# andi611/ZeroSpeech-TTS-without-T

Hardware: AMD Instinct MI355X
Metric: mel-frames/sec (train_ae, seg_len=128, enc_size=1024) (higher is better)
Workload: dtype bf16; 1 GPU; train_ae english hps seg_len=128 enc_size=1024 emb_size=1024 n_speakers=102 F=513, batch=256/GPU, dropout+Gumbel on, fwd+bwd+clip+Adam; global_batch=256, parallelism=dp1

## Files before the change

### include/zs_amd.h

```cpp
#ifndef ZS_AMD_H
#define ZS_AMD_H
#include <stddef.h>
#include <stdint.h>

#ifdef __cplusplus
extern "C" {
#endif

#define ZS_ABI_VERSION 1

enum { ZS_F32 = 0, ZS_BF16 = 1 };
enum { ZS_OK = 0, ZS_EINVAL = -1, ZS_ELAUNCH = -2, ZS_EWORKSPACE = -3 };
enum { ZS_PAD_ZERO = 0, ZS_PAD_REFLECT = 1 };
enum { ZS_ACT_NONE = 0, ZS_ACT_LRELU = 1, ZS_ACT_SIGMOID = 2, ZS_ACT_TANH = 3 };
enum { ZS_STORE_ROWS = 0, ZS_STORE_SPLIT2 = 1 };
enum { ZS_RES_NONE = 0, ZS_RES_IDENTITY = 1, ZS_RES_AVGPOOL2 = 2, ZS_RES_UPSAMPLE2 = 3 };

int zs_abi_version(void);
const char* zs_last_error(void);
int zs_set_option(const char* key, int value);
int zs_get_option(const char* key);

typedef struct {
  int32_t dtype;
// ... 175 lines not shown
  void* out; int64_t ldo; int32_t out_col;
  void* gates;
  float* work; size_t work_bytes;
  int32_t whh_interleaved;
  uint32_t* status;
  const float* bcast_vec; int64_t bcast_ld; const int64_t* bcast_idx; int32_t bcast_col;
  int32_t dir1_forward;
} ZsGruFwd;
size_t zs_gru_work_bytes(int32_t B, int32_t H);
int zs_gru_fwd(const ZsGruFwd* p, void* stream);
int zs_gru_check(const float* work, int32_t B, int32_t H, void* stream);

typedef struct {
  int32_t dtype;
  void* x; int64_t ld; int32_t col0, cols;
  int32_t B, T; const int32_t* lengths;
} ZsRowsReverse;
int zs_rows_reverse(const ZsRowsReverse* p, void* stream);
typedef struct {
  int32_t dtype;
  int32_t B, T, H;
  const void* dout; int64_t ldd; int32_t dout_col;
  const void* out; int64_t ldo; int32_t out_col;
  const void* gates;
  const void* whh_t; int64_t ldw; int32_t n_pad; int64_t w_gstride;
  void* dgi; int64_t ldgi;
  void* dgh; int64_t ldgh;
  float* work; size_t work_bytes;
  uint32_t* status;
} ZsGruBwd;
int zs_gru_bwd(const ZsGruBwd* p, void* stream);
enum { ZS_GRU_PATH_WIDE = 0, ZS_GRU_PATH_PERSIST = 1, ZS_GRU_PATH_STEP_FUSED = 2, ZS_GRU_PATH_STEP_GEMM = 3 };
int zs_gru_path(int32_t pass, int32_t dtype, int32_t B, int32_t T, int32_t H, int32_t whh_interleaved, int32_t wide_aligned);

typedef struct {
  int32_t dtype;
  const float* x_dec; int64_t ld_dec;
  const float* x; int64_t ldx;
  int64_t rows; int32_t F;
  void* dlogits; int64_t ldg; int32_t fill_cols;
  float* partial; float* loss_out; float grad_scale;
} ZsL1Loss;
int zs_l1_loss(const ZsL1Loss* p, void* stream);

int zs_sqnorm(const float* g, int64_t n, double* partial, float* out_sq, void* stream);

typedef struct {
  float* p; float* g; float* m; float* v; int64_t n;
  float lr, beta1, beta2, eps, bc1, bc2;
  const float* sumsq; float max_norm; int32_t write_clipped_grad;
  const int32_t* step_ptr;
  float grad_scale;
  int32_t max_blocks;
  float* ema;
  float ema_decay;
} ZsAdam;
int zs_adam_clip(const ZsAdam* p, void* stream);

int zs_sqnorm_stage1(const float* g, int64_t n, double* partial, void* stream);

enum { ZS_APJ_WEIGHT = 0, ZS_APJ_VECTOR = 1, ZS_APJ_RANGE = 2 };
typedef struct {
  void* dst; int64_t ldw; int64_t dst_elems;
  int32_t transpose, inner_pad, row_offset, col_offset, parity;
  int32_t vlen, src_offset, src_stride;
  const int32_t* row_inv;
// ... 284 lines not shown
```

### zerospeech-tts-without-t_amd/_lib.py

```python
import ctypes
import os
import re

_PKG = os.path.dirname(os.path.abspath(__file__))
_ROOT = os.path.dirname(_PKG)
HEADER = os.path.join(_ROOT, 'include', 'zs_amd.h')
_SAN = os.environ.get('ZS_SANITIZE', '').strip()
LIB_PATH = os.environ.get('ZS_LIB_PATH') or os.path.join(_PKG, 'libzs_amd.%s.so' % _SAN if _SAN else 'libzs_amd.so')

_CTYPES = {
    'int32_t': ctypes.c_int32, 'int64_t': ctypes.c_int64, 'uint32_t': ctypes.c_uint32, 'uint64_t': ctypes.c_uint64,
    'float': ctypes.c_float, 'double': ctypes.c_double, 'size_t': ctypes.c_size_t, 'int': ctypes.c_int,
}


def _strip_comments(text):
    return re.sub(r'/\*.*?\*/', ' ', text, flags=re.S)


def _make_struct(name, fields):
    return type(name, (ctypes.Structure,), {'_fields_': fields})


def parse_header(path=HEADER):
# ... 38 lines not shown


_STRUCT_FIELDS, FUNCTIONS, ENUMS = parse_header()
globals().update(ENUMS)

STRUCTS = {name: _make_struct(name, fields) for name, fields in _STRUCT_FIELDS.items()}
for _fields in _STRUCT_FIELDS.values():
    for _, _ct in _fields:
        _el = getattr(_ct, '_type_', None)
        if isinstance(_el, type) and issubclass(_el, ctypes.Structure):
            STRUCTS[_el.__name__] = _el

_lib = None


class ZsError(RuntimeError):
    pass


def lib():
    global _lib
    if _lib is None:
        if not os.path.exists(LIB_PATH):
            raise ZsError('libzs_amd.so is missing at %s: run `python -c "import __graft_entry__ as g; g.build()"` '
                          '(the HIP extension is mandatory; there is no fallback path)' % LIB_PATH)
        L = ctypes.CDLL(LIB_PATH)
        L.zs_last_error.restype = ctypes.c_char_p
        L.zs_abi_version.restype = ctypes.c_int
        L.zs_gemm_wgrad_workspace_bytes.restype = ctypes.c_size_t
        L.zs_gemm_wgrad_path.argtypes = [ctypes.c_void_p, ctypes.c_void_p, ctypes.c_void_p]
        L.zs_gru_work_bytes.restype = ctypes.c_size_t
        L.zs_gru_work_bytes.argtypes = [ctypes.c_int32, ctypes.c_int32]
        L.zs_gru_check.argtypes = [ctypes.c_void_p, ctypes.c_int32, ctypes.c_int32, ctypes.c_void_p]
        L.zs_sqnorm.argtypes = [ctypes.c_void_p, ctypes.c_int64, ctypes.c_void_p, ctypes.c_void_p, ctypes.c_void_p]
        L.zs_sqnorm_stage1.argtypes = [ctypes.c_void_p, ctypes.c_int64, ctypes.c_void_p, ctypes.c_void_p]
        L.zs_adam_pack_tiles.argtypes = [ctypes.c_void_p]
        L.zs_adam_pack.argtypes = [ctypes.c_void_p, ctypes.c_void_p, ctypes.c_void_p, ctypes.c_int32, ctypes.c_void_p, ctypes.c_int32,
                                   ctypes.c_void_p]
        L.zs_get_option.argtypes = [ctypes.c_char_p]
        L.zs_step_counters.argtypes = [ctypes.c_void_p, ctypes.c_void_p, ctypes.c_void_p]
        L.zs_set_option.argtypes = [ctypes.c_char_p, ctypes.c_int]
        L.zs_pre_mel.argtypes = [ctypes.c_void_p, ctypes.c_void_p, ctypes.c_void_p, ctypes.c_int64, ctypes.c_int32, ctypes.c_float,
                                 ctypes.c_float, ctypes.c_void_p]
        V, I32, I64, F32 = ctypes.c_void_p, ctypes.c_int32, ctypes.c_int64, ctypes.c_float
        L.zs_row_moments_workspace.restype = ctypes.c_size_t
        L.zs_row_moments_workspace.argtypes = [I32, I32, I32]
        L.zs_in2d_finalize.argtypes = [V, V, V, V, I64, I32, F32, V]
        L.zs_in2d_stats.argtypes = [I32, V, I64, I32, I32, I32, F32, V, V, V, ctypes.c_size_t, V]
        L.zs_lerp_rows.argtypes = [V, V, V, V, I32, I64, V]
        L.zs_gp_penalty.argtypes = [V, I32, I64, F32, V, V, V, V]
        L.zs_gen_combine_fwd.argtypes = [V, V, I64, V, I64, I32, I32, V]
        L.zs_l1_plain.argtypes = [V, V, I64, F32, V, V, V, V]
        L.zs_host_fetch.argtypes = [V, V, ctypes.c_size_t, I32, V]
        L.zs_griffin_lim.argtypes = [ctypes.c_void_p, ctypes.c_void_p, ctypes.c_void_p, ctypes.c_int32, ctypes.c_void_p]
        L.zs_conv1_wgrad_workspace.restype = ctypes.c_size_t
        L.zs_conv1_wgrad_workspace.argtypes = []
        L.zs_gl_chains_used.argtypes = []
        L.zs_gl_chains_used.restype = ctypes.c_int
        if hasattr(L, 'zs_gl_denormalize'):
            L.zs_gl_denormalize.argtypes = [ctypes.c_void_p, ctypes.c_void_p, ctypes.c_int64, ctypes.c_void_p]
        if hasattr(L, 'zs_gl_deemphasis'):
            L.zs_gl_deemphasis.argtypes = [ctypes.c_void_p, ctypes.c_int64, ctypes.c_void_p, ctypes.c_int32, ctypes.c_float,
                                           ctypes.c_void_p]
        L.zs_gl_frame_mse.argtypes = [ctypes.c_void_p, ctypes.c_int64, ctypes.c_void_p, ctypes.c_int32, ctypes.c_int32, ctypes.c_int32,
                                      ctypes.c_void_p, ctypes.c_int64, ctypes.c_void_p]
        L.zs_trim_workspace_bytes.restype = ctypes.c_size_t
# ... 111 lines not shown
```

### zerospeech-tts-without-t_amd/csrc/zs_gru.hip

```cpp
#include <stdlib.h>
#include <string.h>

#include <atomic>

#include "zs_common.h"

extern "C" size_t zs_gru_work_bytes(int32_t B, int32_t H);

namespace {

constexpr size_t GRU_WORK_HDR = 256;

constexpr int NTG = 256;

struct GateFwdArgs {
  const void* gi; int64_t ldgi;
  const float* gh;
  const float* bhh; int64_t bhh_gstride;
  float* hstate;
  void* out; int64_t ldo; int out_col;
  void* gates;
  int B, T, H, step;
  int dir1_forward;
};
// ... 657 lines not shown
      }
      if constexpr (NCH > 0) {
        const unsigned poff = (unsigned)(s & 1) * par_bytes;
#pragma unroll
        for (int i = 0; i < NCH; ++i) g4[i] = load16_sc1(hx_rs, poff + ch_off[i]);
      }
      unsigned char* const nimg = &himg[(s + 1) & 1][0];
#pragma unroll
      for (int i = 0; i < 4; ++i) *reinterpret_cast<bf16_t*>(nimg + (4 * q + i) * PITCH + unit * 2) = f2bf(hv[i]);
    }
#pragma unroll
    for (int i = 0; i < 4; ++i) {
      out_s[s & 1][0][4 * q + i][ul] = f2bf(hv[i]);
      out_s[s & 1][1][4 * q + i][ul] = f2bf(rg[i]); out_s[s & 1][2][4 * q + i][ul] = f2bf(zg[i]);
      out_s[s & 1][3][4 * q + i][ul] = f2bf(ng[i]); out_s[s & 1][4][4 * q + i][ul] = f2bf(hn[i]);
    }
  }
  __syncthreads();
  copy_out((T_ - 1) & 1, fwd_t ? T_ - 1 : 0);
}

struct GruPersistBwdArgs {
  const void* dout; int64_t ldd; int dout_col;
  const void* out; int64_t ldo; int out_col;
  const void* gates;
  const void* whh_t; int64_t ldw; int64_t w_gstride;
  void* dgi; int64_t ldgi;
  void* dgh; int64_t ldgh;
  unsigned long long* dx;
  unsigned* err;
  unsigned* status;
  unsigned spin_limit;
  int B, T, H, rows_pad;
};

constexpr int BNT = 4;
template <typename T, int PERB>
__global__ __launch_bounds__(256) void gru_persist_bwd_kernel(const GruPersistBwdArgs a) {
  constexpr int KSTEP = Frag16<T>::KSTEP;
  constexpr int EPL = 16 / (int)sizeof(T);
  constexpr int GPE = 4 / (int)sizeof(T);
  __shared__ float part[4][BNT][4][64];
  const int tid = threadIdx.x, lane = tid & 63, wave = tid >> 6;
  const int q = lane >> 4, r = lane & 15;
  const int d = blockIdx.z, H = a.H, T_ = a.T;
  const int m0 = blockIdx.y * 16;
  const int gpr = 3 * H / GPE;
  const int64_t par_stride = (int64_t)a.rows_pad * gpr;
  unsigned long long* dx_d = a.dx + (int64_t)d * 2 * par_stride;

  uint4 fb[PERB][BNT];
  {
    const T* Wrow = (const T*)a.whh_t + (int64_t)d * a.w_gstride + (int64_t)(blockIdx.x * 16 * BNT + r) * a.ldw + q * EPL;
#pragma unroll
    for (int u = 0; u < PERB; ++u)
#pragma unroll
      for (int c = 0; c < BNT; ++c) fb[u][c] = *reinterpret_cast<const uint4*>(Wrow + (int64_t)(16 * c) * a.ldw + (wave * PERB + u) * KSTEP);
  }
  const bool rvalid = (m0 + r) < a.B;
  const unsigned long long* Ag = dx_d + (int64_t)(m0 + r) * gpr + (q * EPL + wave * PERB * KSTEP) / GPE;
  const int eu2 = tid & 31, e_row = tid >> 5;
  const int j = blockIdx.x * 16 * BNT + 2 * eu2;
  const int hh = (2 * eu2) >> 4, cc = (2 * eu2) & 15;
  float dhd[2][2] = {{0.f, 0.f}, {0.f, 0.f}};
  bool dead = false;

// ... 93 lines not shown
          Pair<T>::publish(xr, j, (unsigned)(s + 1), dr_pre[pz][0], dr_pre[pz][1]);
          Pair<T>::publish(xr, H + j, (unsigned)(s + 1), dz_pre[pz][0], dz_pre[pz][1]);
          Pair<T>::publish(xr, 2 * H + j, (unsigned)(s + 1), dnr[pz][0], dnr[pz][1]);
        }
      }
    }
#pragma unroll
    for (int pz = 0; pz < 2; ++pz) {
      const int b = m0 + e_row + 8 * pz;
      if (b < a.B) {
        const int64_t row = (int64_t)b * T_ + t;
        T* gi = (T*)a.dgi + row * a.ldgi + (int64_t)d * 3 * H + j;
        T* gh = (T*)a.dgh + row * a.ldgh + (int64_t)d * 3 * H + j;
        Pair<T>::st(gi, dr_pre[pz][0], dr_pre[pz][1]); Pair<T>::st(gi + H, dz_pre[pz][0], dz_pre[pz][1]); Pair<T>::st(gi + 2 * H, dn_pre[pz][0], dn_pre[pz][1]);
        Pair<T>::st(gh, dr_pre[pz][0], dr_pre[pz][1]); Pair<T>::st(gh + H, dz_pre[pz][0], dz_pre[pz][1]); Pair<T>::st(gh + 2 * H, dnr[pz][0], dnr[pz][1]);
      }
    }
    __syncthreads();
  }
}

template <int KS>
__global__ __launch_bounds__(256) void gru_wide_bwd_kernel(const GruPersistBwdArgs a) {
  constexpr int H = 32 * KS;
  constexpr int NCH = 3 * (KS / 2 - 1);
  constexpr int NCHA = NCH > 0 ? NCH : 1;
  constexpr int CPR = (H - 64) / 4;
  constexpr int PITCH = 3 * H * 2 + 16;
  __shared__ __attribute__((aligned(16))) unsigned char gimg[2][16 * PITCH];
  __shared__ __attribute__((aligned(16))) bf16_t in_s[2][6][16][64];
  __shared__ __attribute__((aligned(16))) bf16_t out_s[2][4][16][64];
  const int tid = threadIdx.x, lane = tid & 63, wave = tid >> 6;
  const int q = lane >> 4, r = lane & 15;
  const int d = blockIdx.z, T_ = a.T;
  const int m0 = blockIdx.y * 16;
  const int u_wg = blockIdx.x * 64;
  const int ul = wave * 16 + r;
  const int unit = u_wg + ul;
  constexpr int gpr = 3 * H / 2;
  const int64_t par_stride = (int64_t)a.rows_pad * gpr;
  unsigned long long* dx_d = a.dx + (int64_t)d * 2 * par_stride;
  const gru_rsrc_t dx_rs = make_buffer_rsrc(dx_d, (unsigned)(2 * par_stride * 8));
  const unsigned par_bytes = (unsigned)(par_stride * 8);

  uint4 fb[3 * KS];
  {
    const bf16_t* Wb = (const bf16_t*)a.whh_t + (int64_t)d * a.w_gstride + (int64_t)(u_wg + wave * 16 + r) * a.ldw + q * 8;
#pragma unroll
    for (int kk = 0; kk < 3 * KS; ++kk) fb[kk] = *reinterpret_cast<const uint4*>(Wb + kk * 32);
  }
  int ch_row[NCHA], ch_col[NCHA];
  unsigned ch_off[NCHA];
  bool ch_valid[NCHA];
#pragma unroll
  for (int i = 0; i < NCH; ++i) {
    const int c = tid + 256 * i;
    const int row = c / (3 * CPR), rem = c - row * (3 * CPR), g = rem / CPR, cu = (rem - g * CPR) * 4;
    ch_row[i] = row; ch_col[i] = g * H + (cu < u_wg ? cu : cu + 64);
    ch_valid[i] = (m0 + row) < a.B;
    ch_off[i] = (unsigned)(((int64_t)(m0 + row) * gpr + (ch_col[i] >> 1)) * 8);
  }
  auto in_src = [&](int id, int s_) -> const bf16_t* {
    const int arr = id >> 7, rem = id & 127, row = rem >> 3, c = rem & 7;
    const int b = min(m0 + row, a.B - 1);
    const int t = d == 0 ? T_ - 1 - s_ : s_;
    if (arr < 4) return (const bf16_t*)a.gates + (((int64_t)b * T_ + t) * 2 + d) * 4 * H + arr * H + u_wg + 8 * c;
    if (arr == 4) return (const bf16_t*)a.dout + ((int64_t)b * T_ + t) * a.ldd + a.dout_col + d * H + u_wg + 8 * c;
    const int tp = s_ < T_ - 1 ? (d == 0 ? t - 1 : t + 1) : t;
    return (const bf16_t*)a.out + ((int64_t)b * T_ + tp) * a.ldo + a.out_col + d * H + u_wg + 8 * c;
// ... 104 lines not shown
      dnr[i] = dn_pre[i] * r_;
    }
    ZS_PT(3)
    if (s + 1 < T_) {
      unsigned long long* dx_w = dx_d + (int64_t)(s & 1) * par_stride;
#pragma unroll
      for (int i = 0; i < 4; ++i) {
        const float n0 = __shfl_xor(dr_pre[i], 1, 64), n1 = __shfl_xor(dz_pre[i], 1, 64), n2 = __shfl_xor(dnr[i], 1, 64);
        const int b = m0 + 4 * q + i;
        if (!(lane & 1) && b < a.B) {
          unsigned long long* xr = dx_w + (int64_t)b * gpr;
          store_granule(xr + (unit >> 1), (unsigned)(s + 1), Pair<bf16_t>::pack(dr_pre[i], n0));
          store_granule(xr + ((H + unit) >> 1), (unsigned)(s + 1), Pair<bf16_t>::pack(dz_pre[i], n1));
          store_granule(xr + ((2 * H + unit) >> 1), (unsigned)(s + 1), Pair<bf16_t>::pack(dnr[i], n2));
        }
      }
      unsigned char* const nimg = &gimg[(s + 1) & 1][0];
#pragma unroll
      for (int i = 0; i < 4; ++i) {
        bf16_t* row = reinterpret_cast<bf16_t*>(nimg + (4 * q + i) * PITCH);
        row[unit] = f2bf(dr_pre[i]); row[H + unit] = f2bf(dz_pre[i]); row[2 * H + unit] = f2bf(dnr[i]);
      }
    }
#pragma unroll
    for (int i = 0; i < 4; ++i) {
      out_s[s & 1][0][4 * q + i][ul] = f2bf(dr_pre[i]); out_s[s & 1][1][4 * q + i][ul] = f2bf(dz_pre[i]);
      out_s[s & 1][2][4 * q + i][ul] = f2bf(dn_pre[i]); out_s[s & 1][3][4 * q + i][ul] = f2bf(dnr[i]);
    }
    ZS_PT(4)
  }
  __syncthreads();
  copy_out((T_ - 1) & 1, T_ - 1);
#ifdef ZS_GRU_PROFILE
  if (blockIdx.x == 2 && blockIdx.y == 3 && d == 0 && tid == 0) {
    long long* o = reinterpret_cast<long long*>(a.err) + 8;
    for (int k = 0; k < 5; ++k) o[k] = pc[k];
  }
#endif
#undef ZS_PT
}

inline unsigned gate_blocks(int64_t total) {
  int64_t b = (total + NTG - 1) / NTG;
  if (b > 2048) b = 2048;
  return (unsigned)(b < 1 ? 1 : b);
}

size_t gru_hx_bytes(int B, int H, int es) {
  const size_t rows = (size_t)((B + 16 * RB - 1) / (16 * RB)) * 16 * RB;
  return (size_t)2 * 2 * rows * ((size_t)H * es / 4) * 8;
}

Knob g_gru_persist("gru_persist", "ZS_GRU_PERSIST", 1, knob_flag);
Knob g_gru_wide("gru_wide", "ZS_GRU_WIDE", 1, knob_flag);
Knob g_gru_spin_limit("gru_spin_limit", "ZS_GRU_SPIN_LIMIT", (int)GRU_SPIN_LIMIT);
int64_t gru_resident_limit() {
  static std::atomic<int> cus{0};
  int c = cus.load(std::memory_order_relaxed);
  if (c == 0) {
    int dev = 0; hipDeviceProp_t prop;
    if (hipGetDevice(&dev) == hipSuccess && hipGetDeviceProperties(&prop, dev) == hipSuccess) c = prop.multiProcessorCount;
    if (c <= 0) c = 256;
    cus.store(c, std::memory_order_relaxed);
  }
  return c;
}

bool gru_wide_aligned(const ZsGruFwd* p) {
  return (p->out_col % 8) == 0 && (p->ldo % 8) == 0 && (p->ldgi % 8) == 0 && ((uintptr_t)p->out % 16) == 0 && ((uintptr_t)p->gi % 16) == 0 &&
         (!p->gates || ((uintptr_t)p->gates % 16) == 0) && (!p->bcast_vec || (p->bcast_col % 8) == 0);
}
bool gru_wide_aligned(const ZsGruBwd* p) {
  return (p->dout_col % 8) == 0 && (p->out_col % 8) == 0 && (p->ldd % 8) == 0 && (p->ldo % 8) == 0 && (p->ldgi % 8) == 0 && (p->ldgh % 8) == 0 &&
         (((uintptr_t)p->dout | (uintptr_t)p->out | (uintptr_t)p->gates | (uintptr_t)p->dgi | (uintptr_t)p->dgh) % 16) == 0;
}

struct GruPlan {
  int path;
  int per;
  int rb;
  unsigned spin_limit;
};

GruPlan gru_plan(int pass, int dtype, int B, int T, int H, bool whh_interleaved, bool wide_aligned) {
  const bool bwd = pass != 0;
  if (H % 32 != 0 || (!bwd && !whh_interleaved)) return {ZS_GRU_PATH_STEP_GEMM, 0, 0, 0};
  const bool persist = g_gru_persist.get() != 0 && T > 1, wide = g_gru_wide.get() != 0;
  const unsigned spin = (unsigned)g_gru_spin_limit.get();
  const int nrb16 = (B + 15) / 16, nrb = (B + 16 * RB - 1) / (16 * RB);
  const int kstep = dtype == ZS_F32 ? 16 : 32;
  if (persist && wide && dtype == ZS_BF16 && (H == 128 || H == 256 || H == 512) && (int64_t)(H / 64) * nrb16 * 2 <= gru_resident_limit() &&
      wide_aligned)
    return {ZS_GRU_PATH_WIDE, 0, nrb16, spin};
  if (!bwd) {
    const int per = (H % (4 * kstep) == 0) ? H / (4 * kstep) : 0;
    if (persist && (per == 1 || per == 2 || per == 4) && (int64_t)(H / 32) * nrb * 2 <= gru_resident_limit())
      return {ZS_GRU_PATH_PERSIST, per, nrb, spin};
    return {ZS_GRU_PATH_STEP_FUSED, 0, nrb, spin};
  }
  const int perb = ((3 * H) % (4 * kstep) == 0 && H % (16 * BNT) == 0) ? (3 * H) / (4 * kstep) : 0;
  if (persist && (perb == 3 || perb == 6 || perb == 12) && (int64_t)(H / (16 * BNT)) * nrb16 * 2 <= gru_resident_limit())
    return {ZS_GRU_PATH_PERSIST, perb, nrb16, spin};
  return {ZS_GRU_PATH_STEP_FUSED, 0, nrb, spin};
}

GruPlan gru_fwd_plan(const ZsGruFwd* p) {
  return gru_plan(0, p->dtype, p->B, p->T, p->H, p->whh_interleaved != 0, gru_wide_aligned(p));
}

GruPlan gru_bwd_plan(const ZsGruBwd* p) {
  return gru_plan(1, p->dtype, p->B, p->T, p->H, true, gru_wide_aligned(p));
}

}

extern "C" size_t zs_gru_work_bytes(int32_t B, int32_t H) {
  const size_t steps = (size_t)2 * (size_t)B * (size_t)(5 * H) * sizeof(float) + 256;
  const size_t hx = gru_hx_bytes(B, 3 * H, 4) + 256;
  return steps > hx ? steps : hx;
}

extern "C" int zs_gru_check(const float* work, int32_t B, int32_t H, void* stream) {
  ZS_REQUIRE(work && B > 0 && H > 0, "zs_gru_check: bad args");
  unsigned v = 0;
  if (hipMemcpyAsync(&v, reinterpret_cast<const char*>(work), sizeof(v), hipMemcpyDeviceToHost,
                     (hipStream_t)stream) != hipSuccess || hipStreamSynchronize((hipStream_t)stream) != hipSuccess) {
    zs_set_error("zs_gru_check: copy failed");
    return ZS_ELAUNCH;
  }
  if (v != 0) { zs_set_error("zs_gru_check: a persistent GRU workgroup timed out waiting for its group (results are invalid)"); return ZS_ELAUNCH; }
  return ZS_OK;
}

extern "C" int zs_gru_path(int32_t pass, int32_t dtype, int32_t B, int32_t T, int32_t H, int32_t whh_interleaved, int32_t wide_aligned) {
  ZS_REQUIRE(pass == 0 || pass == 1, "zs_gru_path: pass 0 (zs_gru_fwd) or 1 (zs_gru_bwd)");
  ZS_REQUIRE(dtype == ZS_F32 || dtype == ZS_BF16, "zs_gru_path: bad dtype");
  ZS_REQUIRE(B > 0 && T > 0 && H > 0 && H % 8 == 0, "zs_gru_path: sizes");
  const GruPlan pl = gru_plan(pass, dtype, B, T, H, whh_interleaved != 0, wide_aligned != 0);
  return pl.path | (pl.per << 8);
}

extern "C" int zs_gru_fwd(const ZsGruFwd* p, void* stream) {
  ZS_REQUIRE(p && p->gi && p->whh && p->bhh && p->out && p->work, "zs_gru_fwd: null operand");
  ZS_REQUIRE(p->dtype == ZS_F32 || p->dtype == ZS_BF16, "zs_gru_fwd: bad dtype");
  ZS_REQUIRE(p->B > 0 && p->T > 0 && p->H > 0 && p->H % 8 == 0, "zs_gru_fwd: sizes (H %% 8 == 0 required, H=%d)", p->H);
  ZS_REQUIRE(p->work_bytes >= zs_gru_work_bytes(p->B, p->H), "zs_gru_fwd: work buffer too small");
  const int es = p->dtype == ZS_F32 ? 4 : 2;
  const int kc = 128 / es;
  ZS_REQUIRE((p->out_col * es) % 16 == 0, "zs_gru_fwd: out_col alignment");
  const int B = p->B, T = p->T, H = p->H;
  float* const wbase = p->work + GRU_WORK_HDR / sizeof(float);
  float* gh = wbase;
  float* hstate = wbase + (size_t)2 * B * 3 * H;
  const char* outb = (const char*)p->out;
  ZS_REQUIRE(!p->bcast_vec || (p->bcast_idx && (p->bcast_col * es) % 4 == 0), "zs_gru_fwd: bcast_idx / bcast_col");
  const GruPlan pl = gru_fwd_plan(p);
  const bool persistent = pl.path == ZS_GRU_PATH_WIDE || pl.path == ZS_GRU_PATH_PERSIST;
  if (p->bcast_vec && !persistent) {
    ZsAddRowvec r;
    memset(&r, 0, sizeof(r));
    r.dtype = p->dtype; r.vec = p->bcast_vec; r.vec_ld = p->bcast_ld; r.idx = p->bcast_idx;
    r.out = (void*)(outb + (int64_t)p->bcast_col * es); r.ldo = p->ldo; r.B = B; r.T = T; r.C = 2 * H; r.fill_cols = 2 * H;
    int rc = zs_add_rowvec(&r, stream);
    if (rc) return rc;
  }
  if (persistent) {
    GruPersistArgs a;
    memset(&a, 0, sizeof(a));
    a.gi = p->gi; a.ldgi = p->ldgi; a.whh = p->whh; a.ldw = p->ldw; a.w_gstride = p->w_gstride;
    a.bhh = p->bhh; a.bhh_gstride = p->bhh_gstride; a.out = p->out; a.ldo = p->ldo; a.out_col = p->out_col; a.gates = p->gates;
    a.hx = reinterpret_cast<unsigned long long*>(wbase);
    a.err = reinterpret_cast<unsigned*>(p->work);
    a.status = p->status; a.spin_limit = pl.spin_limit;
    a.B = B; a.T = T; a.H = H; a.rows_pad = pl.path == ZS_GRU_PATH_WIDE ? pl.rb * 16 : pl.rb * 16 * RB;
    a.bcast_vec = p->bcast_vec; a.bcast_ld = p->bcast_ld; a.bcast_idx = p->bcast_idx; a.bcast_col = p->bcast_col;
    a.dir1_forward = p->dir1_forward != 0;
    if (hipMemsetAsync(p->work, 0, GRU_WORK_HDR + gru_hx_bytes(B, H, es), (hipStream_t)stream) != hipSuccess) {
      zs_set_error("zs_gru_fwd: memset failed");
      return ZS_ELAUNCH;
    }
    if (pl.path == ZS_GRU_PATH_WIDE) {
      dim3 wgrid(H / 64, pl.rb, 2);
      if (H == 512) hipLaunchKernelGGL(gru_wide_fwd_kernel<16>, wgrid, dim3(256), 0, (hipStream_t)stream, a);
      else if (H == 256) hipLaunchKernelGGL(gru_wide_fwd_kernel<8>, wgrid, dim3(256), 0, (hipStream_t)stream, a);
      else hipLaunchKernelGGL(gru_wide_fwd_kernel<4>, wgrid, dim3(256), 0, (hipStream_t)stream, a);
      return zs_check_launch("zs_gru_fwd.wide");
    }
    dim3 grid(H / 32, pl.rb, 2);
    const int per = pl.per;
#define ZS_GRU_PF(TT, PP) hipLaunchKernelGGL((gru_persist_fwd_kernel<TT, PP>), grid, dim3(256), 0, (hipStream_t)stream, a)
    if (p->dtype == ZS_F32) { if (per == 1) ZS_GRU_PF(float, 1); else if (per == 2) ZS_GRU_PF(float, 2); else ZS_GRU_PF(float, 4); }
    else { if (per == 1) ZS_GRU_PF(bf16_t, 1); else if (per == 2) ZS_GRU_PF(bf16_t, 2); else ZS_GRU_PF(bf16_t, 4); }
#undef ZS_GRU_PF
    return zs_check_launch("zs_gru_fwd.persist");
  }
  if (pl.path == ZS_GRU_PATH_STEP_FUSED) {
    for (int s = 0; s < T; ++s) {
      RowGemmArgs a;
      memset(&a, 0, sizeof(a));
      const int sp = s > 0 ? s - 1 : 0;
      const int64_t off0 = (int64_t)sp * p->ldo + p->out_col;
      const int64_t off1 = (int64_t)(p->dir1_forward ? sp : (s > 0 ? T - s : T - 1)) * p->ldo + p->out_col + H;
      a.A = outb + off0 * es; a.a_row_stride = (int64_t)T * p->ldo; a.a_gstride = off1 - off0;
      a.W = p->whh; a.ldw = p->ldw; a.w_gstride = p->w_gstride;
      a.M = B; a.N = 3 * H; a.K = H;
      GateFwdArgs& g = a.gate;
      g.gi = p->gi; g.ldgi = p->ldgi; g.gh = nullptr; g.bhh = p->bhh; g.bhh_gstride = p->bhh_gstride; g.hstate = hstate;
      g.out = p->out; g.ldo = p->ldo; g.out_col = p->out_col; g.gates = p->gates; g.B = B; g.T = T; g.H = H; g.step = s;
      g.dir1_forward = p->dir1_forward != 0;
// ... 29 lines not shown
    a.dir1_forward = p->dir1_forward != 0;
    const unsigned nb = gate_blocks((int64_t)2 * B * H);
    if (p->dtype == ZS_F32) hipLaunchKernelGGL(gru_gate_fwd_kernel<float>, dim3(nb), dim3(NTG), 0, (hipStream_t)stream, a);
    else hipLaunchKernelGGL(gru_gate_fwd_kernel<bf16_t>, dim3(nb), dim3(NTG), 0, (hipStream_t)stream, a);
    int rc = zs_check_launch("zs_gru_fwd.gate");
    if (rc) return rc;
  }
  return ZS_OK;
}

extern "C" int zs_gru_bwd(const ZsGruBwd* p, void* stream) {
  ZS_REQUIRE(p && p->dout && p->out && p->gates && p->whh_t && p->dgi && p->dgh && p->work, "zs_gru_bwd: null operand");
  ZS_REQUIRE(p->dtype == ZS_F32 || p->dtype == ZS_BF16, "zs_gru_bwd: bad dtype");
  ZS_REQUIRE(p->B > 0 && p->T > 0 && p->H > 0 && p->H % 8 == 0, "zs_gru_bwd: sizes");
  ZS_REQUIRE(p->work_bytes >= zs_gru_work_bytes(p->B, p->H), "zs_gru_bwd: work buffer too small");
  const int es = p->dtype == ZS_F32 ? 4 : 2;
  const int kc = 128 / es;
  const int B = p->B, T = p->T, H = p->H;
  float* const wbase = p->work + GRU_WORK_HDR / sizeof(float);
  float* dhd = wbase + (size_t)2 * B * 3 * H;
  float* dhg = dhd + (size_t)2 * B * H;
  const char* dghb = (const char*)p->dgh;
  const GruPlan pl = gru_bwd_plan(p);
  if (pl.path == ZS_GRU_PATH_WIDE || pl.path == ZS_GRU_PATH_PERSIST) {
    GruPersistBwdArgs a;
    memset(&a, 0, sizeof(a));
    a.dout = p->dout; a.ldd = p->ldd; a.dout_col = p->dout_col; a.out = p->out; a.ldo = p->ldo; a.out_col = p->out_col;
    a.gates = p->gates; a.whh_t = p->whh_t; a.ldw = p->ldw; a.w_gstride = p->w_gstride;
    a.dgi = p->dgi; a.ldgi = p->ldgi; a.dgh = p->dgh; a.ldgh = p->ldgh;
    a.dx = reinterpret_cast<unsigned long long*>(wbase);
    a.err = reinterpret_cast<unsigned*>(p->work);
    a.status = p->status; a.spin_limit = pl.spin_limit;
    a.B = B; a.T = T; a.H = H; a.rows_pad = pl.rb * 16;
    if (hipMemsetAsync(p->work, 0, GRU_WORK_HDR + gru_hx_bytes(B, 3 * H, es), (hipStream_t)stream) != hipSuccess) {
      zs_set_error("zs_gru_bwd: memset failed");
      return ZS_ELAUNCH;
    }
    if (pl.path == ZS_GRU_PATH_WIDE) {
      dim3 wgrid(H / 64, pl.rb, 2);
      if (H == 512) hipLaunchKernelGGL(gru_wide_bwd_kernel<16>, wgrid, dim3(256), 0, (hipStream_t)stream, a);
      else if (H == 256) hipLaunchKernelGGL(gru_wide_bwd_kernel<8>, wgrid, dim3(256), 0, (hipStream_t)stream, a);
      else hipLaunchKernelGGL(gru_wide_bwd_kernel<4>, wgrid, dim3(256), 0, (hipStream_t)stream, a);
      return zs_check_launch("zs_gru_bwd.wide");
    }
    dim3 grid(H / (16 * BNT), pl.rb, 2);
    const int perb = pl.per;
#define ZS_GRU_PB(TT, PP) hipLaunchKernelGGL((gru_persist_bwd_kernel<TT, PP>), grid, dim3(256), 0, (hipStream_t)stream, a)
    if (p->dtype == ZS_F32) { if (perb == 3) ZS_GRU_PB(float, 3); else if (perb == 6) ZS_GRU_PB(float, 6); else ZS_GRU_PB(float, 12); }
    else { if (perb == 3) ZS_GRU_PB(bf16_t, 3); else if (perb == 6) ZS_GRU_PB(bf16_t, 6); else ZS_GRU_PB(bf16_t, 12); }
#undef ZS_GRU_PB
    return zs_check_launch("zs_gru_bwd.persist");
  }
  const bool fast = pl.path == ZS_GRU_PATH_STEP_FUSED;
  for (int s = 0; s < T; ++s) {
    GateBwdArgs a;
    a.dout = p->dout; a.ldd = p->ldd; a.dout_col = p->dout_col; a.out = p->out; a.ldo = p->ldo; a.out_col = p->out_col;
    a.gates = p->gates; a.dhd = dhd; a.dhg = dhg; a.dgi = p->dgi; a.ldgi = p->ldgi; a.dgh = p->dgh; a.ldgh = p->ldgh;
    a.B = B; a.T = T; a.H = H; a.step = s;
    int rc = ZS_OK;
    if (s == 0 || !fast) {
      const unsigned nb = gate_blocks((int64_t)2 * B * H);
      if (p->dtype == ZS_F32) hipLaunchKernelGGL(gru_gate_bwd_kernel<float>, dim3(nb), dim3(NTG), 0, (hipStream_t)stream, a);
      else hipLaunchKernelGGL(gru_gate_bwd_kernel<bf16_t>, dim3(nb), dim3(NTG), 0, (hipStream_t)stream, a);
      rc = zs_check_launch("zs_gru_bwd.gate");
      if (rc) return rc;
    }
    if (s < T - 1 && fast) {
      RowGemmArgs ra;
      memset(&ra, 0, sizeof(ra));
      const int64_t off0 = (int64_t)(T - 1 - s) * p->ldgh;
      const int64_t off1 = (int64_t)s * p->ldgh + 3 * H;
      ra.A = dghb + off0 * es; ra.a_row_stride = (int64_t)T * p->ldgh; ra.a_gstride = off1 - off0;
// ... 28 lines not shown
```

Baseline: 3.162 million frames/s.

## Add single-block GRU kernels for H=128 and XCD-grouped grid for wide backward

Adds solo forward and backward GRU kernels for H=128. Each 16-row batch tile and direction is handled by one workgroup that keeps the recurrent weights in registers and passes the hidden state through LDS, so the cross-block spin synchronization and the workspace memset are no longer needed. It also remaps the wide backward kernel's grid so that blocks sharing a batch tile and direction are grouped, meant to place cooperating blocks on the same XCD and cut cross-die spin latency. The trade-off is far fewer workgroups for H=128 (rb*2 blocks), so each block does four times the MMA work per step.

```diff
diff --git a/include/zs_amd.h b/include/zs_amd.h
--- a/include/zs_amd.h
+++ b/include/zs_amd.h
@@ -231,6 +231,7 @@
 int zs_gru_bwd(const ZsGruBwd* p, void* stream);
 enum { ZS_GRU_PATH_WIDE = 0, ZS_GRU_PATH_PERSIST = 1, ZS_GRU_PATH_STEP_FUSED = 2, ZS_GRU_PATH_STEP_GEMM = 3 };
 int zs_gru_path(int32_t pass, int32_t dtype, int32_t B, int32_t T, int32_t H, int32_t whh_interleaved, int32_t wide_aligned);
+int zs_gru_solo(int32_t pass, int32_t dtype, int32_t B, int32_t T, int32_t H, int32_t whh_interleaved, int32_t wide_aligned);
 
 typedef struct {
   int32_t dtype;
diff --git a/zerospeech-tts-without-t_amd/_lib.py b/zerospeech-tts-without-t_amd/_lib.py
--- a/zerospeech-tts-without-t_amd/_lib.py
+++ b/zerospeech-tts-without-t_amd/_lib.py
@@ -94,6 +94,7 @@
         L.zs_gru_work_bytes.restype = ctypes.c_size_t
         L.zs_gru_work_bytes.argtypes = [ctypes.c_int32, ctypes.c_int32]
         L.zs_gru_check.argtypes = [ctypes.c_void_p, ctypes.c_int32, ctypes.c_int32, ctypes.c_void_p]
+        L.zs_gru_solo.argtypes = [ctypes.c_int32] * 7
         L.zs_sqnorm.argtypes = [ctypes.c_void_p, ctypes.c_int64, ctypes.c_void_p, ctypes.c_void_p, ctypes.c_void_p]
         L.zs_sqnorm_stage1.argtypes = [ctypes.c_void_p, ctypes.c_int64, ctypes.c_void_p, ctypes.c_void_p]
         L.zs_adam_pack_tiles.argtypes = [ctypes.c_void_p]
diff --git a/zerospeech-tts-without-t_amd/csrc/zs_gru.hip b/zerospeech-tts-without-t_amd/csrc/zs_gru.hip
--- a/zerospeech-tts-without-t_amd/csrc/zs_gru.hip
+++ b/zerospeech-tts-without-t_amd/csrc/zs_gru.hip
@@ -713,6 +713,7 @@
   unsigned* status;
   unsigned spin_limit;
   int B, T, H, rows_pad;
+  int xcd_groups;
 };
 
 constexpr int BNT = 4;
@@ -872,9 +873,9 @@
   __shared__ __attribute__((aligned(16))) bf16_t out_s[2][4][16][64];
   const int tid = threadIdx.x, lane = tid & 63, wave = tid >> 6;
   const int q = lane >> 4, r = lane & 15;
-  const int d = blockIdx.z, T_ = a.T;
-  const int m0 = blockIdx.y * 16;
-  const int u_wg = blockIdx.x * 64;
+  const int d = a.xcd_groups ? (int)(blockIdx.x & 1) : (int)blockIdx.z, T_ = a.T;
+  const int m0 = (a.xcd_groups ? (int)(blockIdx.x >> 1) : (int)blockIdx.y) * 16;
+  const int u_wg = (a.xcd_groups ? (int)blockIdx.y : (int)blockIdx.x) * 64;
   const int ul = wave * 16 + r;
   const int unit = u_wg + ul;
   constexpr int gpr = 3 * H / 2;
@@ -1045,12 +1046,245 @@
   __syncthreads();
   copy_out((T_ - 1) & 1, T_ - 1);
 #ifdef ZS_GRU_PROFILE
-  if (blockIdx.x == 2 && blockIdx.y == 3 && d == 0 && tid == 0) {
+  if (u_wg == 128 && m0 == 48 && d == 0 && tid == 0) {
     long long* o = reinterpret_cast<long long*>(a.err) + 8;
     for (int k = 0; k < 5; ++k) o[k] = pc[k];
   }
 #endif
 #undef ZS_PT
+}
+
+constexpr int SOLO_H = 128;
+constexpr int SOLO_KS = SOLO_H / 32;
+constexpr int SOLO_HP = SOLO_H + 8;
+
+__global__ __launch_bounds__(256) void gru_solo_fwd_kernel(const GruPersistArgs a) {
+  constexpr int H = SOLO_H, KS = SOLO_KS;
+  constexpr int PITCH = H * 2 + 16;
+  __shared__ __attribute__((aligned(16))) unsigned char himg[2][16 * PITCH];
+  __shared__ __attribute__((aligned(16))) bf16_t gi_s[2][16][3][SOLO_HP];
+  __shared__ __attribute__((aligned(16))) bf16_t out_s[2][5][16][SOLO_HP];
+  __shared__ __attribute__((aligned(16))) bf16_t bc_s[16][SOLO_HP];
+  const int tid = threadIdx.x, lane = tid & 63, wave = tid >> 6;
+  const int q = lane >> 4, r = lane & 15;
+  const int d = blockIdx.z, T_ = a.T;
+  const int m0 = blockIdx.y * 16;
+
+  uint4 fb[2][KS][3];
+  {
+    const bf16_t* Wb = (const bf16_t*)a.whh + (int64_t)d * a.w_gstride + (int64_t)(wave * 96 + r) * a.ldw + q * 8;
+#pragma unroll
+    for (int tl = 0; tl < 2; ++tl)
+#pragma unroll
+      for (int ks = 0; ks < KS; ++ks)
+#pragma unroll
+        for (int g = 0; g < 3; ++g) fb[tl][ks][g] = *reinterpret_cast<const uint4*>(Wb + (int64_t)(32 * g + 16 * tl) * a.ldw + ks * 32);
+  }
+  const float* bh = a.bhh + (int64_t)d * a.bhh_gstride;
+  int unit[2];
+  float b_r[2], b_z[2], b_n[2];
+#pragma unroll
+  for (int tl = 0; tl < 2; ++tl) {
+    unit[tl] = wave * 32 + tl * 16 + r;
+    b_r[tl] = bh[unit[tl]]; b_z[tl] = bh[H + unit[tl]]; b_n[tl] = bh[2 * H + unit[tl]];
+  }
+  auto gi_src = [&](int id, int t) -> const bf16_t* {
+    const int row = id / 48, rem = id - row * 48, g = rem >> 4, c = rem & 15;
+    const int b = min(m0 + row, a.B - 1);
+    return (const bf16_t*)a.gi + ((int64_t)b * T_ + t) * a.ldgi + (int64_t)d * 3 * H + g * H + 8 * c;
+  };
+  auto gi_dst = [&](int par, int id) -> uint4* {
+    const int row = id / 48, rem = id - row * 48, g = rem >> 4, c = rem & 15;
+    return reinterpret_cast<uint4*>(&gi_s[par][row][g][8 * c]);
+  };
+  auto copy_out = [&](int par, int t) {
+#pragma unroll
+    for (int k = 0; k < 6; ++k) {
+      const int row = tid >> 4, c = tid & 15;
+      const int b = m0 + row;
+      if (b >= a.B) continue;
+      if (k == 0) {
+        *reinterpret_cast<uint4*>((bf16_t*)a.out + ((int64_t)b * T_ + t) * a.ldo + a.out_col + d * H + 8 * c) =
+            *reinterpret_cast<const uint4*>(&out_s[par][0][row][8 * c]);
+      } else if (k < 5) {
+        if (a.gates)
+          *reinterpret_cast<uint4*>((bf16_t*)a.gates + (((int64_t)b * T_ + t) * 2 + d) * 4 * H + (k - 1) * H + 8 * c) =
+              *reinterpret_cast<const uint4*>(&out_s[par][k][row][8 * c]);
+      } else if (a.bcast_vec) {
+        *reinterpret_cast<uint4*>((bf16_t*)a.out + ((int64_t)b * T_ + t) * a.ldo + a.bcast_col + d * H + 8 * c) =
+            *reinterpret_cast<const uint4*>(&bc_s[row][8 * c]);
+      }
+    }
+  };
+  float hp[2][4] = {{0.f, 0.f, 0.f, 0.f}, {0.f, 0.f, 0.f, 0.f}};
+  if (a.bcast_vec) {
+#pragma unroll
+    for (int tl = 0; tl < 2; ++tl)
+#pragma unroll
+      for (int i = 0; i < 4; ++i) {
+        const int b = min(m0 + 4 * q + i, a.B - 1);
+        bc_s[4 * q + i][unit[tl]] = f2bf(a.bcast_vec[a.bcast_idx[b] * a.bcast_ld + d * H + unit[tl]]);
+      }
+  }
+  const bool fwd_t = d == 0 || a.dir1_forward;
+  uint4 gq0 = *reinterpret_cast<const uint4*>(gi_src(tid, fwd_t ? 0 : T_ - 1));
+  uint4 gq1 = *reinterpret_cast<const uint4*>(gi_src(tid + 256, fwd_t ? 0 : T_ - 1));
+  uint4 gq2 = *reinterpret_cast<const uint4*>(gi_src(tid + 512, fwd_t ? 0 : T_ - 1));
+
+  for (int s = 0; s < T_; ++s) {
+    const unsigned char* const img = &himg[s & 1][0];
+    f32x4_t acc[2][3];
+#pragma unroll
+    for (int tl = 0; tl < 2; ++tl)
+#pragma unroll
+      for (int g = 0; g < 3; ++g) acc[tl][g] = f32x4_t{0.f, 0.f, 0.f, 0.f};
+    *gi_dst(s & 1, tid) = gq0; *gi_dst(s & 1, tid + 256) = gq1; *gi_dst(s & 1, tid + 512) = gq2;
+    __syncthreads();
+    if (s > 0) copy_out((s - 1) & 1, fwd_t ? s - 1 : T_ - s);
+    if (s + 1 < T_) {
+      const int tn = fwd_t ? s + 1 : T_ - 2 - s;
+      gq0 = *reinterpret_cast<const uint4*>(gi_src(tid, tn));
+      gq1 = *reinterpret_cast<const uint4*>(gi_src(tid + 256, tn));
+      gq2 = *reinterpret_cast<const uint4*>(gi_src(tid + 512, tn));
+    }
+    if (s > 0) {
+#pragma unroll
+      for (int ks = 0; ks < KS; ++ks) {
+        const uint4 fa = *reinterpret_cast<const uint4*>(img + r * PITCH + q * 16 + ks * 64);
+#pragma unroll
+        for (int tl = 0; tl < 2; ++tl)
+#pragma unroll
+          for (int g = 0; g < 3; ++g) Frag16<bf16_t>::mma(fa, fb[tl][ks][g], acc[tl][g]);
+      }
+    }
+    unsigned char* const nimg = &himg[(s + 1) & 1][0];
+#pragma unroll
+    for (int tl = 0; tl < 2; ++tl) {
+      const int ul = unit[tl];
+#pragma unroll
+      for (int i = 0; i < 4; ++i) {
+        const float gi_r = bf2f(gi_s[s & 1][4 * q + i][0][ul]), gi_z = bf2f(gi_s[s & 1][4 * q + i][1][ul]), gi_n = bf2f(gi_s[s & 1][4 * q + i][2][ul]);
+        const float rg = 1.f / (1.f + expf(-(gi_r + (acc[tl][0][i] + b_r[tl]))));
+        const float zg = 1.f / (1.f + expf(-(gi_z + (acc[tl][1][i] + b_z[tl]))));
+        const float hn = acc[tl][2][i] + b_n[tl];
+        const float ng = tanhf(gi_n + rg * hn);
+        const float hv = __builtin_fmaf(zg, hp[tl][i], (1.f - zg) * ng);
+        hp[tl][i] = hv;
+        const bf16_t hb = f2bf(hv);
+        if (s + 1 < T_) *reinterpret_cast<bf16_t*>(nimg + (4 * q + i) * PITCH + ul * 2) = hb;
+        out_s[s & 1][0][4 * q + i][ul] = hb;
+        out_s[s & 1][1][4 * q + i][ul] = f2bf(rg); out_s[s & 1][2][4 * q + i][ul] = f2bf(zg);
+        out_s[s & 1][3][4 * q + i][ul] = f2bf(ng); out_s[s & 1][4][4 * q + i][ul] = f2bf(hn);
+      }
+    }
+  }
+  __syncthreads();
+  copy_out((T_ - 1) & 1, fwd_t ? T_ - 1 : 0);
+}
+
+__global__ __launch_bounds__(256) void gru_solo_bwd_kernel(const GruPersistBwdArgs a) {
+  constexpr int H = SOLO_H, KS = SOLO_KS;
+  constexpr int PITCH = 3 * H * 2 + 16;
+  __shared__ __attribute__((aligned(16))) unsigned char gimg[2][16 * PITCH];
+  __shared__ __attribute__((aligned(16))) bf16_t in_s[2][6][16][SOLO_HP];
+  __shared__ __attribute__((aligned(16))) bf16_t dn_s[2][16][SOLO_HP];
+  const int tid = threadIdx.x, lane = tid & 63, wave = tid >> 6;
+  const int q = lane >> 4, r = lane & 15;
+  const int d = blockIdx.z, T_ = a.T;
+  const int m0 = blockIdx.y * 16;
+
+  uint4 fb[2][3 * KS];
+  int unit[2];
+#pragma unroll
+  for (int tl = 0; tl < 2; ++tl) {
+    unit[tl] = wave * 32 + tl * 16 + r;
+    const bf16_t* Wb = (const bf16_t*)a.whh_t + (int64_t)d * a.w_gstride + (int64_t)unit[tl] * a.ldw + q * 8;
+#pragma unroll
+    for (int kk = 0; kk < 3 * KS; ++kk) fb[tl][kk] = *reinterpret_cast<const uint4*>(Wb + kk * 32);
+  }
+  const int x_row = tid >> 4, x_c = tid & 15;
+  auto in_src = [&](int arr, int s_) -> const bf16_t* {
+    const int b = min(m0 + x_row, a.B - 1);
+    const int t = d == 0 ? T_ - 1 - s_ : s_;
+    if (arr < 4) return (const bf16_t*)a.gates + (((int64_t)b * T_ + t) * 2 + d) * 4 * H + arr * H + 8 * x_c;
+    if (arr == 4) return (const bf16_t*)a.dout + ((int64_t)b * T_ + t) * a.ldd + a.dout_col + d * H + 8 * x_c;
+    const int tp = s_ < T_ - 1 ? (d == 0 ? t - 1 : t + 1) : t;
+    return (const bf16_t*)a.out + ((int64_t)b * T_ + tp) * a.ldo + a.out_col + d * H + 8 * x_c;
+  };
+  auto copy_out = [&](int s_) {
+    const int t = d == 0 ? T_ - 1 - s_ : s_;
+    const int b = m0 + x_row;
+    if (b >= a.B) return;
+    const unsigned char* const grow = &gimg[(s_ + 1) & 1][0] + x_row * PITCH;
+#pragma unroll
+    for (int arr = 0; arr < 6; ++arr) {
+      const int g = arr < 3 ? arr : arr - 3;
+      bf16_t* base = arr < 3 ? (bf16_t*)a.dgi + ((int64_t)b * T_ + t) * a.ldgi : (bf16_t*)a.dgh + ((int64_t)b * T_ + t) * a.ldgh;
+      const uint4 v = arr == 2 ? *reinterpret_cast<const uint4*>(&dn_s[s_ & 1][x_row][8 * x_c])
+                               : *reinterpret_cast<const uint4*>(grow + (g * H + 8 * x_c) * 2);
+      *reinterpret_cast<uint4*>(base + (int64_t)d * 3 * H + g * H + 8 * x_c) = v;
+    }
+  };
+  uint4 gq[6];
+#pragma unroll
+  for (int k = 0; k < 6; ++k) gq[k] = *reinterpret_cast<const uint4*>(in_src(k, 0));
+  float dhd[2][4] = {{0.f, 0.f, 0.f, 0.f}, {0.f, 0.f, 0.f, 0.f}};
+
+  for (int s = 0; s < T_; ++s) {
+    const unsigned char* const img = &gimg[s & 1][0];
+    f32x4_t acc[2][3];
+#pragma unroll
+    for (int tl = 0; tl < 2; ++tl)
+#pragma unroll
+      for (int g = 0; g < 3; ++g) acc[tl][g] = f32x4_t{0.f, 0.f, 0.f, 0.f};
+#pragma unroll
+    for (int k = 0; k < 6; ++k) {
+      uint4 v = gq[k];
+      if (k == 5 && s == T_ - 1) v = make_uint4(0, 0, 0, 0);
+      *reinterpret_cast<uint4*>(&in_s[s & 1][k][x_row][8 * x_c]) = v;
+    }
+    __syncthreads();
+    if (s > 0) copy_out(s - 1);
+    if (s + 1 < T_) {
+#pragma unroll
+      for (int k = 0; k < 6; ++k) gq[k] = *reinterpret_cast<const uint4*>(in_src(k, s + 1));
+    }
+    if (s > 0) {
+#pragma unroll
+      for (int ks = 0; ks < KS; ++ks)
+#pragma unroll
+        for (int g = 0; g < 3; ++g) {
+          const uint4 fa = *reinterpret_cast<const uint4*>(img + r * PITCH + q * 16 + (g * KS + ks) * 64);
+#pragma unroll
+          for (int tl = 0; tl < 2; ++tl) Frag16<bf16_t>::mma(fa, fb[tl][g * KS + ks], acc[tl][g]);
+        }
+    }
+    unsigned char* const nimg = &gimg[(s + 1) & 1][0];
+#pragma unroll
+    for (int tl = 0; tl < 2; ++tl) {
+      const int ul = unit[tl];
+#pragma unroll
+      for (int i = 0; i < 4; ++i) {
+        const int row = 4 * q + i;
+        const float r_ = bf2f(in_s[s & 1][0][row][ul]), z_ = bf2f(in_s[s & 1][1][row][ul]), n_ = bf2f(in_s[s & 1][2][row][ul]);
+        const float hn_ = bf2f(in_s[s & 1][3][row][ul]), do_ = bf2f(in_s[s & 1][4][row][ul]), hp_ = bf2f(in_s[s & 1][5][row][ul]);
+        float dh = do_ + dhd[tl][i];
+        if (s > 0) dh += (acc[tl][0][i] + acc[tl][1][i]) + acc[tl][2][i];
+        const float dn = dh * (1.f - z_);
+        const float dz = dh * (hp_ - n_);
+        dhd[tl][i] = dh * z_;
+        const float dn_pre = dn * (1.f - n_ * n_);
+        const float dr_pre = dn_pre * hn_ * r_ * (1.f - r_);
+        const float dz_pre = dz * z_ * (1.f - z_);
+        const float dnr = dn_pre * r_;
+        bf16_t* irow = reinterpret_cast<bf16_t*>(nimg + row * PITCH);
+        irow[ul] = f2bf(dr_pre); irow[H + ul] = f2bf(dz_pre); irow[2 * H + ul] = f2bf(dnr);
+        dn_s[s & 1][row][ul] = f2bf(dn_pre);
+      }
+    }
+  }
+  __syncthreads();
+  copy_out(T_ - 1);
 }
 
 inline unsigned gate_blocks(int64_t total) {
@@ -1067,6 +1301,8 @@
 Knob g_gru_persist("gru_persist", "ZS_GRU_PERSIST", 1, knob_flag);
 Knob g_gru_wide("gru_wide", "ZS_GRU_WIDE", 1, knob_flag);
 Knob g_gru_spin_limit("gru_spin_limit", "ZS_GRU_SPIN_LIMIT", (int)GRU_SPIN_LIMIT);
+Knob g_gru_xcd_groups("gru_xcd_groups", "ZS_GRU_XCD_GROUPS", 1);
+Knob g_gru_solo_max_h("gru_solo_max_h", "ZS_GRU_SOLO_MAX_H", SOLO_H);
 int64_t gru_resident_limit() {
   static std::atomic<int> cus{0};
   int c = cus.load(std::memory_order_relaxed);
@@ -1093,28 +1329,31 @@
   int per;
   int rb;
   unsigned spin_limit;
+  bool solo;
 };
 
 GruPlan gru_plan(int pass, int dtype, int B, int T, int H, bool whh_interleaved, bool wide_aligned) {
   const bool bwd = pass != 0;
-  if (H % 32 != 0 || (!bwd && !whh_interleaved)) return {ZS_GRU_PATH_STEP_GEMM, 0, 0, 0};
+  if (H % 32 != 0 || (!bwd && !whh_interleaved)) return {ZS_GRU_PATH_STEP_GEMM, 0, 0, 0, false};
   const bool persist = g_gru_persist.get() != 0 && T > 1, wide = g_gru_wide.get() != 0;
   const unsigned spin = (unsigned)g_gru_spin_limit.get();
   const int nrb16 = (B + 15) / 16, nrb = (B + 16 * RB - 1) / (16 * RB);
   const int kstep = dtype == ZS_F32 ? 16 : 32;
   if (persist && wide && dtype == ZS_BF16 && (H == 128 || H == 256 || H == 512) && (int64_t)(H / 64) * nrb16 * 2 <= gru_resident_limit() &&
-      wide_aligned)
-    return {ZS_GRU_PATH_WIDE, 0, nrb16, spin};
+      wide_aligned) {
+    const bool solo = H == SOLO_H && H <= g_gru_solo_max_h.get() && spin != 0;
+    return {ZS_GRU_PATH_WIDE, 0, nrb16, spin, solo};
+  }
   if (!bwd) {
     const int per = (H % (4 * kstep) == 0) ? H / (4 * kstep) : 0;
     if (persist && (per == 1 || per == 2 || per == 4) && (int64_t)(H / 32) * nrb * 2 <= gru_resident_limit())
-      return {ZS_GRU_PATH_PERSIST, per, nrb, spin};
-    return {ZS_GRU_PATH_STEP_FUSED, 0, nrb, spin};
+      return {ZS_GRU_PATH_PERSIST, per, nrb, spin, false};
+    return {ZS_GRU_PATH_STEP_FUSED, 0, nrb, spin, false};
   }
   const int perb = ((3 * H) % (4 * kstep) == 0 && H % (16 * BNT) == 0) ? (3 * H) / (4 * kstep) : 0;
   if (persist && (perb == 3 || perb == 6 || perb == 12) && (int64_t)(H / (16 * BNT)) * nrb16 * 2 <= gru_resident_limit())
-    return {ZS_GRU_PATH_PERSIST, perb, nrb16, spin};
-  return {ZS_GRU_PATH_STEP_FUSED, 0, nrb, spin};
+    return {ZS_GRU_PATH_PERSIST, perb, nrb16, spin, false};
+  return {ZS_GRU_PATH_STEP_FUSED, 0, nrb, spin, false};
 }
 
 GruPlan gru_fwd_plan(const ZsGruFwd* p) {
@@ -1151,6 +1390,13 @@
   ZS_REQUIRE(B > 0 && T > 0 && H > 0 && H % 8 == 0, "zs_gru_path: sizes");
   const GruPlan pl = gru_plan(pass, dtype, B, T, H, whh_interleaved != 0, wide_aligned != 0);
   return pl.path | (pl.per << 8);
+}
+
+extern "C" int zs_gru_solo(int32_t pass, int32_t dtype, int32_t B, int32_t T, int32_t H, int32_t whh_interleaved, int32_t wide_aligned) {
+  ZS_REQUIRE(pass == 0 || pass == 1, "zs_gru_solo: pass 0 (zs_gru_fwd) or 1 (zs_gru_bwd)");
+  ZS_REQUIRE(dtype == ZS_F32 || dtype == ZS_BF16, "zs_gru_solo: bad dtype");
+  ZS_REQUIRE(B > 0 && T > 0 && H > 0 && H % 8 == 0, "zs_gru_solo: sizes");
+  return gru_plan(pass, dtype, B, T, H, whh_interleaved != 0, wide_aligned != 0).solo ? 1 : 0;
 }
 
 extern "C" int zs_gru_fwd(const ZsGruFwd* p, void* stream) {
@@ -1188,6 +1434,10 @@
     a.B = B; a.T = T; a.H = H; a.rows_pad = pl.path == ZS_GRU_PATH_WIDE ? pl.rb * 16 : pl.rb * 16 * RB;
     a.bcast_vec = p->bcast_vec; a.bcast_ld = p->bcast_ld; a.bcast_idx = p->bcast_idx; a.bcast_col = p->bcast_col;
     a.dir1_forward = p->dir1_forward != 0;
+    if (pl.solo) {
+      hipLaunchKernelGGL(gru_solo_fwd_kernel, dim3(1, pl.rb, 2), dim3(256), 0, (hipStream_t)stream, a);
+      return zs_check_launch("zs_gru_fwd.solo");
+    }
     if (hipMemsetAsync(p->work, 0, GRU_WORK_HDR + gru_hx_bytes(B, H, es), (hipStream_t)stream) != hipSuccess) {
       zs_set_error("zs_gru_fwd: memset failed");
       return ZS_ELAUNCH;
@@ -1283,12 +1533,18 @@
     a.err = reinterpret_cast<unsigned*>(p->work);
     a.status = p->status; a.spin_limit = pl.spin_limit;
     a.B = B; a.T = T; a.H = H; a.rows_pad = pl.rb * 16;
+    if (pl.solo) {
+      hipLaunchKernelGGL(gru_solo_bwd_kernel, dim3(1, pl.rb, 2), dim3(256), 0, (hipStream_t)stream, a);
+      return zs_check_launch("zs_gru_bwd.solo");
+    }
     if (hipMemsetAsync(p->work, 0, GRU_WORK_HDR + gru_hx_bytes(B, 3 * H, es), (hipStream_t)stream) != hipSuccess) {
       zs_set_error("zs_gru_bwd: memset failed");
       return ZS_ELAUNCH;
     }
     if (pl.path == ZS_GRU_PATH_WIDE) {
       dim3 wgrid(H / 64, pl.rb, 2);
+      a.xcd_groups = g_gru_xcd_groups.get() != 0 && (pl.rb * 2) % 8 == 0;
+      if (a.xcd_groups) wgrid = dim3(pl.rb * 2, H / 64, 1);
       if (H == 512) hipLaunchKernelGGL(gru_wide_bwd_kernel<16>, wgrid, dim3(256), 0, (hipStream_t)stream, a);
       else if (H == 256) hipLaunchKernelGGL(gru_wide_bwd_kernel<8>, wgrid, dim3(256), 0, (hipStream_t)stream, a);
       else hipLaunchKernelGGL(gru_wide_bwd_kernel<4>, wgrid, dim3(256), 0, (hipStream_t)stream, a);
```

Result: faster. 3.216 million frames/s (median of 6 runs) (+1.7%).
